# facebookresearch/jepa

Hardware: NVIDIA H100
Metric: clips/sec ViT-L/16 16x224^2 synthetic V-JEPA pre-training step (higher is better)
Workload: dtype bf16

## Files before the change

jepa_b200/csrc/attn_bwd.cu:

```cuda
#include <stdlib.h>

#include "attn_common.cuh"
#include "vjepa_b200.h"

namespace vj {

constexpr int kBwdThreads = 256;
constexpr int kBwdStream = 64;

struct AttnBwdParams {
  const int* cu_seqlens;
  const float* lse2;
  const float* delta;
  __nv_bfloat16* dqkv;
  int H, T;
  float scale, scale_log2;
};

template <int HD>
struct BwdCfg {
  using A = AttnCfg<HD>;
  static constexpr int RES = A::template tile_bytes<128>();
  static constexpr int STR = A::template tile_bytes<kBwdStream>();
  static constexpr int T0 = 0, T1 = RES;
  static constexpr int S_OFF = 2 * RES;
  static constexpr int BAR_OFF = S_OFF + 4 * STR;
  static constexpr int SMEM_BYTES = BAR_OFF + 64 + 1024;
};

__global__ void __launch_bounds__(256) attn_delta_kernel(const __nv_bfloat16* __restrict__ o,
                                                         const __nv_bfloat16* __restrict__ dout,
                                                         float* __restrict__ delta, int T, int H, int HD) {
  const int lane = threadIdx.x & 31;
  const int wpb = blockDim.x >> 5;
  const int D = H * HD;
  const int nvec = D >> 3;
  const int lanes_per_head = HD >> 3;
  for (long long t = (long long)blockIdx.x * wpb + (threadIdx.x >> 5); t < T; t += (long long)gridDim.x * wpb) {
    for (int c = lane; c < ((nvec + 31) / 32) * 32; c += 32) {
      float s = 0.f;
      if (c < nvec) {
        const uint4 a = *reinterpret_cast<const uint4*>(o + t * D + c * 8);
        const uint4 b = *reinterpret_cast<const uint4*>(dout + t * D + c * 8);
        s = bf16_lo(a.x) * bf16_lo(b.x) + bf16_hi(a.x) * bf16_hi(b.x) + bf16_lo(a.y) * bf16_lo(b.y) +
            bf16_hi(a.y) * bf16_hi(b.y) + bf16_lo(a.z) * bf16_lo(b.z) + bf16_hi(a.z) * bf16_hi(b.z) +
            bf16_lo(a.w) * bf16_lo(b.w) + bf16_hi(a.w) * bf16_hi(b.w);
      }
      for (int o2 = lanes_per_head >> 1; o2 > 0; o2 >>= 1) s += __shfl_xor_sync(0xffffffffu, s, o2);
      if (c < nvec && (lane % lanes_per_head) == 0) delta[(long long)((c * 8) / HD) * T + t] = s;
    }
  }
}

template <int HD, bool DKV>
__global__ void __launch_bounds__(kBwdThreads, 1)
attn_bwd_kernel(const __grid_constant__ CUtensorMap tmRes, const __grid_constant__ CUtensorMap tmStr,
                const __grid_constant__ CUtensorMap tmDO, const AttnBwdParams p) {
  using B = BwdCfg<HD>;
  extern __shared__ uint8_t smem_raw[];
  uint8_t* smem = reinterpret_cast<uint8_t*>((reinterpret_cast<uintptr_t>(smem_raw) + 1023) & ~uintptr_t(1023));

  const int seq = blockIdx.y, head = blockIdx.z;
  const int row_begin = p.cu_seqlens[seq];
  const int len = p.cu_seqlens[seq + 1] - row_begin;
  const int t0 = blockIdx.x * 128;
  if (t0 >= len) return;
  const int n_it = (len + kBwdStream - 1) / kBwdStream;
  const int HHD = p.H * HD;

  uint64_t* bars = reinterpret_cast<uint64_t*>(smem + B::BAR_OFF);
  const uint32_t bar_res = smem_u32(bars + 0);
  const uint32_t bar_s0 = smem_u32(bars + 1);
  const uint32_t sT0 = smem_u32(smem + B::T0), sT1 = smem_u32(smem + B::T1), sS = smem_u32(smem + B::S_OFF);

  auto load_stream = [&](int i) {
    const int st = i & 1;
    const uint32_t a = sS + st * 2 * B::STR, b = a + B::STR, bar = bar_s0 + 8 * st;
    const int r0 = row_begin + i * kBwdStream;
    mbar_expect_tx(bar, 2 * B::STR);
    if (DKV) {
      attn_load_tile<HD, kBwdStream>(a, &tmStr, bar, head * HD, r0);
      attn_load_tile<HD, kBwdStream>(b, &tmDO, bar, head * HD, r0);
    } else {
      attn_load_tile<HD, kBwdStream>(a, &tmStr, bar, HHD + head * HD, r0);
      attn_load_tile<HD, kBwdStream>(b, &tmStr, bar, 2 * HHD + head * HD, r0);
    }
  };
  if (threadIdx.x == 0) {
    mbar_init(bar_res, 1);
    mbar_init(bar_s0, 1);
    mbar_init(bar_s0 + 8, 1);
    fence_mbar_init();
    mbar_expect_tx(bar_res, 2 * B::RES);
    if (DKV) {
      attn_load_tile<HD, 128>(sT0, &tmRes, bar_res, HHD + head * HD, row_begin + t0);
      attn_load_tile<HD, 128>(sT1, &tmRes, bar_res, 2 * HHD + head * HD, row_begin + t0);
    } else {
      attn_load_tile<HD, 128>(sT0, &tmRes, bar_res, head * HD, row_begin + t0);
      attn_load_tile<HD, 128>(sT1, &tmDO, bar_res, head * HD, row_begin + t0);
    }
    load_stream(0);
    if (n_it > 1) load_stream(1);
  }
  __syncthreads();

  const int wg = threadIdx.x >> 7;
  const int lane = threadIdx.x & 31;
  const int r = wg * 64 + ((threadIdx.x >> 5) & 3) * 16 + (lane >> 2);
  const float* lse_h = p.lse2 + (long long)head * p.T + row_begin;
  const float* del_h = p.delta + (long long)head * p.T + row_begin;
  float acc0[HD / 2], acc1[HD / 2];
#pragma unroll
  for (int i = 0; i < HD / 2; ++i) { acc0[i] = 0.f; acc1[i] = 0.f; }
  float row_lse[2], row_del[2];
  if (!DKV) {
#pragma unroll
    for (int h = 0; h < 2; ++h) {
      const int q = t0 + r + 8 * h;
      row_lse[h] = q < len ? lse_h[q] : 0.f;
      row_del[h] = q < len ? del_h[q] : 0.f;
    }
  }

  mbar_wait(bar_res, 0);
  for (int i = 0; i < n_it; ++i) {
    const int st = i & 1;
    const uint32_t sa = sS + st * 2 * B::STR, sb = sa + B::STR;
    const int c0 = i * kBwdStream;
    mbar_wait(bar_s0 + 8 * st, (i >> 1) & 1);
    float x[kBwdStream / 2], y[kBwdStream / 2];
    wgmma_fence();
#pragma unroll
    for (int kk = 0; kk < HD / 16; ++kk)
      wgmma_ss<kBwdStream, 0, 0>(x, attn_kmajor_desc<HD, 128>(sT0, wg * 64, kk), attn_kmajor_desc<HD, kBwdStream>(sa, 0, kk),
                                 kk > 0);
#pragma unroll
    for (int kk = 0; kk < HD / 16; ++kk)
      wgmma_ss<kBwdStream, 0, 0>(y, attn_kmajor_desc<HD, 128>(sT1, wg * 64, kk), attn_kmajor_desc<HD, kBwdStream>(sb, 0, kk),
                                 kk > 0);
    wgmma_commit();
    wgmma_wait<0>();
    wgmma_fence_regs(x);
    wgmma_fence_regs(y);

#pragma unroll
    for (int c = 0; c < kBwdStream / 8; ++c)
#pragma unroll
      for (int e = 0; e < 2; ++e) {
        const int col = c0 + 8 * c + 2 * (lane & 3) + e;
        const bool col_ok = col < len;
        float cl = 0.f, cd = 0.f;
        if (DKV && col_ok) { cl = lse_h[col]; cd = del_h[col]; }
#pragma unroll
        for (int h = 0; h < 2; ++h) {
          const float l2 = DKV ? cl : row_lse[h], dl = DKV ? cd : row_del[h];
          float& pv = x[4 * c + 2 * h + e];
          float& dv = y[4 * c + 2 * h + e];
          pv = col_ok ? ex2_approx(fmaf(pv, p.scale_log2, -l2)) : 0.f;
          dv = pv * (dv - dl);
        }
      }

    wgmma_fence_regs(acc0);
    wgmma_fence_regs(acc1);
    wgmma_fence();
#pragma unroll
    for (int kk = 0; kk < kBwdStream / 16; ++kk) {
      uint32_t a[4];
      if (DKV) {
        acc_to_afrag(x, kk, a);
        wgmma_rs<HD, 1>(acc0, a, attn_mnmajor_desc<HD, kBwdStream>(sb, kk), 1);
        acc_to_afrag(y, kk, a);
        wgmma_rs<HD, 1>(acc1, a, attn_mnmajor_desc<HD, kBwdStream>(sa, kk), 1);
      } else {
        acc_to_afrag(y, kk, a);
        wgmma_rs<HD, 1>(acc0, a, attn_mnmajor_desc<HD, kBwdStream>(sa, kk), 1);
      }
    }
    wgmma_commit();
    wgmma_wait<0>();
    wgmma_fence_regs(acc0);
    wgmma_fence_regs(acc1);
    __syncthreads();
    if (threadIdx.x == 0 && i + 2 < n_it) load_stream(i + 2);
  }

  __nv_bfloat16* rows = p.dqkv + (long long)(row_begin + t0) * 3 * HHD + head * HD;
  if (DKV) {
    store_frag_bf16<HD>(acc1, p.scale, rows + HHD, 3LL * HHD, r, len - t0);
    store_frag_bf16<HD>(acc0, 1.0f, rows + 2 * HHD, 3LL * HHD, r, len - t0);
  } else {
    store_frag_bf16<HD>(acc0, p.scale, rows, 3LL * HHD, r, len - t0);
  }
}

template <int HD>
static int launch_attn_bwd(const void* qkv, const void* out, const void* dout, const float* lse2, float* delta,
                           void* dqkv, const int* cu, int nseq, int max_len, int H, int T, float scale, cudaStream_t s) {
  using C = AttnCfg<HD>;
  using B = BwdCfg<HD>;
  CUtensorMap tq128, tq64, tdo128, tdo64;
  const uint64_t W = (uint64_t)3 * H * HD;
  int rc = make_tmap_2d(&tq128, qkv, 0, W, T, W * 2, C::BOX_INNER, 128, C::TMAP_SWIZZLE);
  if (!rc) rc = make_tmap_2d(&tq64, qkv, 0, W, T, W * 2, C::BOX_INNER, kBwdStream, C::TMAP_SWIZZLE);
  if (!rc) rc = make_tmap_2d(&tdo128, dout, 0, (uint64_t)H * HD, T, (uint64_t)H * HD * 2, C::BOX_INNER, 128, C::TMAP_SWIZZLE);
  if (!rc) rc = make_tmap_2d(&tdo64, dout, 0, (uint64_t)H * HD, T, (uint64_t)H * HD * 2, C::BOX_INNER, kBwdStream,
                             C::TMAP_SWIZZLE);
  if (rc) return rc;
  auto kdkv = attn_bwd_kernel<HD, true>;
  auto kdq = attn_bwd_kernel<HD, false>;
  static bool configured = false;
  if (!configured) {
    VJ_CUDA(cudaFuncSetAttribute(kdkv, cudaFuncAttributeMaxDynamicSharedMemorySize, B::SMEM_BYTES));
    VJ_CUDA(cudaFuncSetAttribute(kdq, cudaFuncAttributeMaxDynamicSharedMemorySize, B::SMEM_BYTES));
    configured = true;
  }
  {
    int g = (T + 7) / 8;
    const int cap = num_sms() * 8;
    if (g > cap) g = cap;
    attn_delta_kernel<<<g, 256, 0, s>>>(reinterpret_cast<const __nv_bfloat16*>(out),
                                        reinterpret_cast<const __nv_bfloat16*>(dout), delta, T, H, HD);
    VJ_CUDA(cudaGetLastError());
    vj::count_launch(1);
  }
  AttnBwdParams p;
  p.cu_seqlens = cu; p.lse2 = lse2; p.delta = delta; p.dqkv = reinterpret_cast<__nv_bfloat16*>(dqkv);
  p.H = H; p.T = T; p.scale = scale; p.scale_log2 = scale * 1.4426950408889634f;
  dim3 grid((max_len + 127) / 128, nseq, H);
  kdkv<<<grid, kBwdThreads, B::SMEM_BYTES, s>>>(tq128, tq64, tdo64, p);
  VJ_CUDA(cudaGetLastError());
  kdq<<<grid, kBwdThreads, B::SMEM_BYTES, s>>>(tq128, tq64, tdo128, p);
  VJ_CUDA(cudaGetLastError());
  vj::count_launch(2);
  return 0;
}

// ... 18 lines not shown
```

jepa_b200/csrc/attn_fwd.cu:

```cuda
#include <stdlib.h>

#include "attn_common.cuh"
#include "vjepa_b200.h"

namespace vj {

constexpr int kFwdThreads = 256;
constexpr int kFwdKV = 128;

struct AttnFwdParams {
  const int* cu_seqlens;
  __nv_bfloat16* out;
  float* lse2;
  int H, T;
  long long ld_out;
  float scale_log2;
};

template <int HD>
struct FwdCfg {
  using A = AttnCfg<HD>;
  static constexpr int TILE = A::template tile_bytes<128>();
  static constexpr int Q_OFF = 0;
  static constexpr int K_OFF = TILE;
  static constexpr int V_OFF = 3 * TILE;
  static constexpr int BAR_OFF = 5 * TILE;
  static constexpr int SMEM_BYTES = BAR_OFF + 64 + 1024;
};

template <int HD>
__global__ void __launch_bounds__(kFwdThreads, 1)
attn_fwd_kernel(const __grid_constant__ CUtensorMap tmQKV, const AttnFwdParams p) {
  using F = FwdCfg<HD>;
  extern __shared__ uint8_t smem_raw[];
  uint8_t* smem = reinterpret_cast<uint8_t*>((reinterpret_cast<uintptr_t>(smem_raw) + 1023) & ~uintptr_t(1023));

  const int seq = blockIdx.y, head = blockIdx.z;
  const int row_begin = p.cu_seqlens[seq];
  const int len = p.cu_seqlens[seq + 1] - row_begin;
  const int q0 = blockIdx.x * 128;
  if (q0 >= len) return;
  const int n_kv = (len + kFwdKV - 1) / kFwdKV;

  uint64_t* bars = reinterpret_cast<uint64_t*>(smem + F::BAR_OFF);
  const uint32_t bar_q = smem_u32(bars + 0);
  const uint32_t bar_kv0 = smem_u32(bars + 1);
  const uint32_t sQ = smem_u32(smem + F::Q_OFF), sK = smem_u32(smem + F::K_OFF), sV = smem_u32(smem + F::V_OFF);
  const int HHD = p.H * HD;

  auto load_kv = [&](int j) {
    const int st = j & 1;
    mbar_expect_tx(bar_kv0 + 8 * st, 2 * F::TILE);
    attn_load_tile<HD, 128>(sK + st * F::TILE, &tmQKV, bar_kv0 + 8 * st, HHD + head * HD, row_begin + j * kFwdKV);
    attn_load_tile<HD, 128>(sV + st * F::TILE, &tmQKV, bar_kv0 + 8 * st, 2 * HHD + head * HD, row_begin + j * kFwdKV);
  };
  if (threadIdx.x == 0) {
    mbar_init(bar_q, 1);
    mbar_init(bar_kv0, 1);
    mbar_init(bar_kv0 + 8, 1);
    fence_mbar_init();
    tma_prefetch_desc(&tmQKV);
    mbar_expect_tx(bar_q, F::TILE);
    attn_load_tile<HD, 128>(sQ, &tmQKV, bar_q, head * HD, row_begin + q0);
    load_kv(0);
    if (n_kv > 1) load_kv(1);
  }
  __syncthreads();

  const int wg = threadIdx.x >> 7;
  const int lane = threadIdx.x & 31;
  const int r = wg * 64 + ((threadIdx.x >> 5) & 3) * 16 + (lane >> 2);
  float o[HD / 2];
#pragma unroll
  for (int i = 0; i < HD / 2; ++i) o[i] = 0.f;
  float m_run[2] = {-INFINITY, -INFINITY}, l_run[2] = {0.f, 0.f};

  mbar_wait(bar_q, 0);
  for (int j = 0; j < n_kv; ++j) {
    const int st = j & 1;
    const int valid = min(kFwdKV, len - j * kFwdKV);
    mbar_wait(bar_kv0 + 8 * st, (j >> 1) & 1);
    float s[kFwdKV / 2];
    wgmma_fence();
#pragma unroll
    for (int kk = 0; kk < HD / 16; ++kk)
      wgmma_ss<kFwdKV, 0, 0>(s, attn_kmajor_desc<HD, 128>(sQ, wg * 64, kk),
                             attn_kmajor_desc<HD, 128>(sK + st * F::TILE, 0, kk), kk > 0);
    wgmma_commit();
    wgmma_wait<0>();
    wgmma_fence_regs(s);

    float alpha[2];
#pragma unroll
    for (int h = 0; h < 2; ++h) {
      float mx = -INFINITY;
#pragma unroll
      for (int c = 0; c < kFwdKV / 8; ++c)
#pragma unroll
        for (int e = 0; e < 2; ++e) {
          const int key = 8 * c + 2 * (lane & 3) + e;
          float& v = s[4 * c + 2 * h + e];
          if (key >= valid) v = -INFINITY;
          mx = fmaxf(mx, v);
        }
      mx = quad_max(mx);
      const float m_new = fmaxf(m_run[h], mx);
      alpha[h] = ex2_approx((m_run[h] - m_new) * p.scale_log2);
      m_run[h] = m_new;
      const float moff = m_new * p.scale_log2;
      float sum = 0.f;
#pragma unroll
      for (int c = 0; c < kFwdKV / 8; ++c)
#pragma unroll
        for (int e = 0; e < 2; ++e) {
          float& v = s[4 * c + 2 * h + e];
          v = ex2_approx(fmaf(v, p.scale_log2, -moff));
          sum += v;
        }
      l_run[h] = l_run[h] * alpha[h] + sum;
    }
#pragma unroll
    for (int c = 0; c < HD / 8; ++c) {
      o[4 * c + 0] *= alpha[0]; o[4 * c + 1] *= alpha[0];
      o[4 * c + 2] *= alpha[1]; o[4 * c + 3] *= alpha[1];
    }

    wgmma_fence_regs(o);
    wgmma_fence();
#pragma unroll
    for (int kk = 0; kk < kFwdKV / 16; ++kk) {
      uint32_t a[4];
      acc_to_afrag(s, kk, a);
      wgmma_rs<HD, 1>(o, a, attn_mnmajor_desc<HD, 128>(sV + st * F::TILE, kk), 1);
    }
    wgmma_commit();
    wgmma_wait<0>();
    wgmma_fence_regs(o);
    __syncthreads();
    if (threadIdx.x == 0 && j + 2 < n_kv) load_kv(j + 2);
  }

  float inv[2];
#pragma unroll
  for (int h = 0; h < 2; ++h) {
    const float l = quad_sum(l_run[h]);
    inv[h] = 1.0f / l;
    const int row = q0 + r + 8 * h;
    if ((lane & 3) == 0 && row < len) p.lse2[(long long)head * p.T + row_begin + row] = m_run[h] * p.scale_log2 + log2f(l);
  }
#pragma unroll
  for (int c = 0; c < HD / 8; ++c) {
    o[4 * c + 0] *= inv[0]; o[4 * c + 1] *= inv[0];
    o[4 * c + 2] *= inv[1]; o[4 * c + 3] *= inv[1];
  }
  store_frag_bf16<HD>(o, 1.0f, p.out + (long long)(row_begin + q0) * p.ld_out + head * HD, p.ld_out, r, len - q0);
}

template <int HD>
static int launch_attn_fwd(const void* qkv, void* out, float* lse2, const int* cu, int nseq, int max_len, int H, int T,
                           float scale, cudaStream_t s) {
  using C = AttnCfg<HD>;
  using F = FwdCfg<HD>;
  CUtensorMap tm;
  int rc = make_tmap_2d(&tm, qkv, 0, (uint64_t)3 * H * HD, T, (uint64_t)3 * H * HD * 2, C::BOX_INNER, 128,
                        C::TMAP_SWIZZLE);
  if (rc) return rc;
  auto kern = attn_fwd_kernel<HD>;
  static bool configured = false;
  if (!configured) {
    VJ_CUDA(cudaFuncSetAttribute(kern, cudaFuncAttributeMaxDynamicSharedMemorySize, F::SMEM_BYTES));
    configured = true;
  }
  AttnFwdParams p;
  p.cu_seqlens = cu; p.out = reinterpret_cast<__nv_bfloat16*>(out); p.lse2 = lse2;
  p.H = H; p.T = T; p.ld_out = (long long)H * HD;
  p.scale_log2 = scale * 1.4426950408889634f;
  dim3 grid((max_len + 127) / 128, nseq, H);
  kern<<<grid, kFwdThreads, F::SMEM_BYTES, s>>>(tm, p);
  VJ_CUDA(cudaGetLastError());
  vj::count_launch(1);
  return 0;
}

}

extern "C" int vj_attn_fwd(const void* qkv, void* out, float* lse2, const int* cu_seqlens, int nseq, int max_len,
                           int H, int HD, int T, float scale, void* stream_) {
  using namespace vj;
  cudaStream_t s = reinterpret_cast<cudaStream_t>(stream_);
  VJ_CHECK_ARG(qkv && out && lse2 && cu_seqlens, "vj_attn_fwd: null pointer");
  VJ_CHECK_ARG(nseq > 0 && max_len > 0 && H > 0 && T > 0, "vj_attn_fwd: empty problem");
  VJ_CHECK_ARG((reinterpret_cast<uintptr_t>(qkv) & 15) == 0 && (reinterpret_cast<uintptr_t>(out) & 15) == 0,
               "vj_attn_fwd: pointers must be 16-byte aligned");
// ... 8 lines not shown
```

jepa_b200/csrc/common.cuh:

```cuda
#pragma once

#include <cuda.h>
#include <cuda_bf16.h>
#include <cuda_runtime.h>
#include <stdint.h>

#ifndef VJ_DEVINL
#define VJ_DEVINL __device__ __forceinline__
#endif

namespace vj {

void set_error(const char* fmt, ...);
int cuda_fail(cudaError_t e, const char* what);

#define VJ_CHECK_ARG(cond, ...)                 \
  do {                                          \
    if (!(cond)) {                              \
      vj::set_error(__VA_ARGS__);               \
      return -1;                                \
    }                                           \
  } while (0)

#define VJ_CUDA(expr)                                         \
  do {                                                        \
    cudaError_t _e = (expr);                                  \
    if (_e != cudaSuccess) return vj::cuda_fail(_e, #expr);   \
  } while (0)

int num_sms();
int sm_budget();
void count_launch(int n);

int make_tmap_2d(CUtensorMap* out, const void* ptr, int dtype, uint64_t inner, uint64_t outer,
                 uint64_t ld_bytes, uint32_t box_inner, uint32_t box_outer, int swizzle);

VJ_DEVINL uint32_t smem_u32(const void* p) {
  return static_cast<uint32_t>(__cvta_generic_to_shared(p));
}

VJ_DEVINL void mbar_init(uint32_t bar, uint32_t count) {
  asm volatile("mbarrier.init.shared::cta.b64 [%0], %1;" ::"r"(bar), "r"(count) : "memory");
}
VJ_DEVINL void fence_mbar_init() {
  asm volatile("fence.mbarrier_init.release.cluster;" ::: "memory");
}
VJ_DEVINL void fence_proxy_async_smem() {
  asm volatile("fence.proxy.async.shared::cta;" ::: "memory");
}
VJ_DEVINL void mbar_expect_tx(uint32_t bar, uint32_t bytes) {
  asm volatile("mbarrier.arrive.expect_tx.shared::cta.b64 _, [%0], %1;" ::"r"(bar), "r"(bytes)
               : "memory");
}
VJ_DEVINL void mbar_arrive(uint32_t bar) {
  asm volatile("mbarrier.arrive.shared::cta.b64 _, [%0];" ::"r"(bar) : "memory");
}
VJ_DEVINL bool mbar_try_wait(uint32_t bar, uint32_t parity) {
  uint32_t ok;
  asm volatile(
      "{\n\t.reg .pred p;\n\t"
      "mbarrier.try_wait.parity.shared::cta.b64 p, [%1], %2;\n\t"
      "selp.u32 %0, 1, 0, p;\n\t}"
      : "=r"(ok)
      : "r"(bar), "r"(parity)
      : "memory");
  return ok != 0;
}
VJ_DEVINL void mbar_wait(uint32_t bar, uint32_t parity) {
  while (!mbar_try_wait(bar, parity)) {
  }
}

VJ_DEVINL void tma_prefetch_desc(const CUtensorMap* m) {
  asm volatile("prefetch.tensormap [%0];" ::"l"(reinterpret_cast<uint64_t>(m)) : "memory");
}
VJ_DEVINL void tma_load_2d(uint32_t smem_dst, const CUtensorMap* m, uint32_t bar, int c0, int c1) {
  asm volatile(
      "cp.async.bulk.tensor.2d.shared::cluster.global.mbarrier::complete_tx::bytes [%0], [%1, {%3, %4}], [%2];"
      ::"r"(smem_dst), "l"(reinterpret_cast<uint64_t>(m)), "r"(bar), "r"(c0), "r"(c1)
      : "memory");
}
VJ_DEVINL void tma_store_2d(const CUtensorMap* m, uint32_t smem_src, int c0, int c1) {
  asm volatile("cp.async.bulk.tensor.2d.global.shared::cta.bulk_group [%0, {%2, %3}], [%1];" ::"l"(
                   reinterpret_cast<uint64_t>(m)),
               "r"(smem_src), "r"(c0), "r"(c1)
               : "memory");
}
VJ_DEVINL void tma_reduce_add_2d(const CUtensorMap* m, uint32_t smem_src, int c0, int c1) {
  asm volatile(
      "cp.reduce.async.bulk.tensor.2d.global.shared::cta.add.tile.bulk_group [%0, {%2, %3}], [%1];" ::"l"(
          reinterpret_cast<uint64_t>(m)),
      "r"(smem_src), "r"(c0), "r"(c1)
      : "memory");
}
VJ_DEVINL void tma_commit_group() { asm volatile("cp.async.bulk.commit_group;" ::: "memory"); }
template <int N>
VJ_DEVINL void tma_wait_group_read() {
  asm volatile("cp.async.bulk.wait_group.read %0;" ::"n"(N) : "memory");
}
template <int N>
VJ_DEVINL void tma_wait_group() {
  asm volatile("cp.async.bulk.wait_group %0;" ::"n"(N) : "memory");
}

VJ_DEVINL void sts128(uint32_t addr, const uint4& v) {
  asm volatile("st.shared.v4.b32 [%0], {%1, %2, %3, %4};" ::"r"(addr), "r"(v.x), "r"(v.y), "r"(v.z), "r"(v.w) : "memory");
}
VJ_DEVINL void sts128f(uint32_t addr, const float4& v) {
  asm volatile("st.shared.v4.f32 [%0], {%1, %2, %3, %4};" ::"r"(addr), "f"(v.x), "f"(v.y), "f"(v.z), "f"(v.w) : "memory");
}
VJ_DEVINL uint4 lds128(uint32_t addr) {
  uint4 v;
  asm volatile("ld.shared.v4.b32 {%0, %1, %2, %3}, [%4];" : "=r"(v.x), "=r"(v.y), "=r"(v.z), "=r"(v.w) : "r"(addr) : "memory");
  return v;
}
VJ_DEVINL float4 lds128f(uint32_t addr) {
  float4 v;
  asm volatile("ld.shared.v4.f32 {%0, %1, %2, %3}, [%4];" : "=f"(v.x), "=f"(v.y), "=f"(v.z), "=f"(v.w) : "r"(addr) : "memory");
  return v;
}
VJ_DEVINL void sts32f(uint32_t addr, float v) { asm volatile("st.shared.f32 [%0], %1;" ::"r"(addr), "f"(v) : "memory"); }
VJ_DEVINL float lds32f(uint32_t addr) {
  float v;
  asm volatile("ld.shared.f32 %0, [%1];" : "=f"(v) : "r"(addr) : "memory");
// ... 51 lines not shown
```

jepa_b200/csrc/gemm.cu:

```cuda

#include <stdlib.h>

#include "common.cuh"
#include "vjepa_b200.h"
#include "wgmma.cuh"

namespace vj {

constexpr int BM = 128;
constexpr int BK = 64;
constexpr int kGemmThreads = 384;
constexpr int kPromoteKB = 4;

struct GemmParams {
  int M, N, K;
  int tiles_m, tiles_n, split_k, kb_total, kb_per_split;
  int stream_k;
  long long sk_chunk;
  const float* bias;
  int epi;
  const void* aux;
  long long ldaux;
  const int* aux_rowmap;
  int aux_period;
// ... 23 lines not shown
  WorkCursor c;
  if (p.stream_k) {
    const long long total_kb = (long long)p.tiles_m * p.tiles_n * p.kb_total;
    c.cur = (long long)blockIdx.x * p.sk_chunk;
    c.end = min(total_kb, c.cur + p.sk_chunk);
  } else {
    c.cur = blockIdx.x;
    c.end = (long long)p.tiles_m * p.tiles_n * p.split_k;
  }
  return c;
}
VJ_DEVINL bool work_next(const GemmParams& p, WorkCursor& c, int& t, int& kb0, int& kb1) {
  if (c.cur >= c.end) return false;
  if (p.stream_k) {
    t = int(c.cur / p.kb_total);
    kb0 = int(c.cur - (long long)t * p.kb_total);
    const long long take = min((long long)(p.kb_total - kb0), c.end - c.cur);
    kb1 = kb0 + int(take);
    c.cur += take;
  } else {
    const int tiles = p.tiles_m * p.tiles_n;
    const int split = int(c.cur / tiles);
    t = int(c.cur - (long long)split * tiles);
    kb0 = split * p.kb_per_split;
    kb1 = min(p.kb_total, kb0 + p.kb_per_split);
    c.cur += gridDim.x;
  }
  return true;
}

VJ_DEVINL float erf_as(float x) {
  const float ax = fabsf(x);
  const float t = __fdividef(1.0f, fmaf(0.3275911f, ax, 1.0f));
  float poly = fmaf(1.061405429f, t, -1.453152027f);
  poly = fmaf(poly, t, 1.421413741f);
  poly = fmaf(poly, t, -0.284496736f);
  poly = fmaf(poly, t, 0.254829592f);
  poly *= t;
  const float r = 1.0f - poly * __expf(-ax * ax);
  return copysignf(r, x);
}
VJ_DEVINL float gelu_and_grad(float x, float& d) {
  const float cdf = 0.5f * (1.0f + erf_as(x * 0.70710678118654752f));
  const float pdf = 0.39894228040143268f * __expf(-0.5f * x * x);
  d = fmaf(x, pdf, cdf);
  return x * cdf;
}
VJ_DEVINL float gelu_grad_fast(float x) {
  float d;
  gelu_and_grad(x, d);
  return d;
}

VJ_DEVINL void setmaxnreg_dec40() { asm volatile("setmaxnreg.dec.sync.aligned.u32 40;"); }
VJ_DEVINL void setmaxnreg_inc232() { asm volatile("setmaxnreg.inc.sync.aligned.u32 232;"); }

template <int BN, bool A_MN, bool B_MN, bool OUT_F32, int EPI, bool AUX32>
__global__ void __launch_bounds__(kGemmThreads, 1)
gemm_kernel(const __grid_constant__ CUtensorMap tmA, const __grid_constant__ CUtensorMap tmB, const GemmParams p) {
  constexpr bool kUsesAux = (EPI == VJ_EPI_ADD || EPI == VJ_EPI_DGELU || EPI == VJ_EPI_MUL);
  using Cfg = GemmCfg<BN>;
  constexpr int STAGES = Cfg::STAGES;
  extern __shared__ uint8_t smem_raw[];
  uint8_t* smem = reinterpret_cast<uint8_t*>((reinterpret_cast<uintptr_t>(smem_raw) + 1023) & ~uintptr_t(1023));
  uint64_t* bars = reinterpret_cast<uint64_t*>(smem + Cfg::BAR_OFF);
  const uint32_t full0 = smem_u32(bars);
  const uint32_t empty0 = smem_u32(bars + STAGES);
  const int wg = threadIdx.x >> 7;

  if (threadIdx.x == 0) {
    for (int s = 0; s < STAGES; ++s) {
      mbar_init(full0 + 8 * s, 1);
      mbar_init(empty0 + 8 * s, 8);
    }
    fence_mbar_init();
    tma_prefetch_desc(&tmA);
    tma_prefetch_desc(&tmB);
  }
  __syncthreads();

  if (wg == 0) {
    setmaxnreg_dec40();
    if (threadIdx.x == 0) {
      int stage = 0;
      uint32_t phase = 0;
      WorkCursor wc = work_begin(p);
      int t, kb0, kb1;
      while (work_next(p, wc, t, kb0, kb1)) {
        const int m0 = (t / p.tiles_n) * BM;
        const int n0 = (t % p.tiles_n) * BN;
        for (int kb = kb0; kb < kb1; ++kb) {
          mbar_wait(empty0 + 8 * stage, phase ^ 1);
          const uint32_t sa = smem_u32(smem + stage * Cfg::STAGE_BYTES);
          const uint32_t sb = sa + Cfg::A_BYTES;
          const uint32_t fb = full0 + 8 * stage;
          mbar_expect_tx(fb, Cfg::STAGE_BYTES);
          const int k0 = kb * BK;
          if (!A_MN) {
            tma_load_2d(sa, &tmA, fb, k0, m0);
          } else {
#pragma unroll
            for (int j = 0; j < BM / 64; ++j) tma_load_2d(sa + j * 8192, &tmA, fb, m0 + 64 * j, k0);
          }
          if (!B_MN) {
            tma_load_2d(sb, &tmB, fb, k0, n0);
          } else {
#pragma unroll
            for (int j = 0; j < BN / 64; ++j) tma_load_2d(sb + j * 8192, &tmB, fb, n0 + 64 * j, k0);
          }
          if (++stage == STAGES) {
            stage = 0;
            phase ^= 1;
          }
        }
      }
    }
    return;
  }

  setmaxnreg_inc232();
  const int cw = wg - 1;
  const int warp_in_wg = (threadIdx.x >> 5) & 3;
  const int lane = threadIdx.x & 31;
  constexpr bool kPromote = A_MN && B_MN;
  static_assert(!kPromote || BN <= 128, "promoted accumulation needs two accumulator sets in registers");
  int stage = 0;
  uint32_t phase = 0;
  float acc[BN / 2];
  float part[kPromote ? BN / 2 : 1];
  WorkCursor wc = work_begin(p);
  int t, kb0, kb1;
  while (work_next(p, wc, t, kb0, kb1)) {
    const int m0 = (t / p.tiles_n) * BM;
    const int n0 = (t % p.tiles_n) * BN;
    if constexpr (kPromote) {
#pragma unroll
      for (int i = 0; i < BN / 2; ++i) acc[i] = 0.f;
    }
    int prev = -1;
    for (int kb = kb0; kb < kb1; ++kb) {
      mbar_wait(full0 + 8 * stage, phase);
      const uint32_t sa = smem_u32(smem + stage * Cfg::STAGE_BYTES) + cw * 8192;
      const uint32_t sb = smem_u32(smem + stage * Cfg::STAGE_BYTES) + Cfg::A_BYTES;
      const uint64_t da0 = A_MN ? make_smem_desc(sa, 8192, 1024, 1) : make_smem_desc(sa, 16, 1024, 1);
      const uint64_t db0 = B_MN ? make_smem_desc(sb, 8192, 1024, 1) : make_smem_desc(sb, 16, 1024, 1);
      if constexpr (kPromote) {
        const bool group_first = (kb - kb0) % kPromoteKB == 0;
        const bool group_last = (kb - kb0) % kPromoteKB == kPromoteKB - 1 || kb + 1 == kb1;
        wgmma_fence_regs(part);
        wgmma_fence();
#pragma unroll
        for (int kk = 0; kk < BK / 16; ++kk)
          wgmma_ss<BN, 1, 1>(part, da0 + ((kk * 2048) >> 4), db0 + ((kk * 2048) >> 4), (!group_first || kk > 0) ? 1 : 0);
        wgmma_commit();
        if (group_last) {
          wgmma_wait<0>();
          wgmma_fence_regs(part);
#pragma unroll
          for (int i = 0; i < BN / 2; ++i) acc[i] += part[i];
        } else {
          wgmma_wait<1>();
        }
      } else {
        wgmma_fence_regs(acc);
        wgmma_fence();
#pragma unroll
        for (int kk = 0; kk < BK / 16; ++kk) {
          const uint32_t koa = A_MN ? kk * 2048 : kk * 32, kob = B_MN ? kk * 2048 : kk * 32;
          wgmma_ss<BN, A_MN ? 1 : 0, B_MN ? 1 : 0>(acc, da0 + (koa >> 4), db0 + (kob >> 4), (kb > kb0 || kk > 0) ? 1 : 0);
        }
        wgmma_commit();
        wgmma_wait<1>();
        wgmma_fence_regs(acc);
// ... 200 lines not shown
```

jepa_b200/csrc/wgmma.cuh:

```cuda
#pragma once
#include <stdint.h>

namespace vj {

__device__ __forceinline__ void wgmma_fence() { asm volatile("wgmma.fence.sync.aligned;" ::: "memory"); }
__device__ __forceinline__ void wgmma_commit() { asm volatile("wgmma.commit_group.sync.aligned;" ::: "memory"); }
template <int N>
__device__ __forceinline__ void wgmma_wait() { asm volatile("wgmma.wait_group.sync.aligned %0;" ::"n"(N) : "memory"); }
template <int R>
__device__ __forceinline__ void wgmma_fence_regs(float (&d)[R]) {
#pragma unroll
  for (int i = 0; i < R; ++i) asm volatile("" : "+f"(d[i])::"memory");
}

template <int N, int TA, int TB>
__device__ __forceinline__ void wgmma_ss(float (&d)[N / 2], uint64_t da, uint64_t db, int scale_d);
template <int N, int TB>
__device__ __forceinline__ void wgmma_rs(float (&d)[N / 2], const uint32_t (&a)[4], uint64_t db, int scale_d);

#define VJ_WGMMA_SS_64(TA, TB)                                                                                   \
  template <>                                                                                                    \
  __device__ __forceinline__ void wgmma_ss<64, TA, TB>(float (&d)[32], uint64_t da, uint64_t db, int scale_d) {   \
    asm volatile("{\n.reg .pred p;\nsetp.ne.b32 p, %34, 0;\n"                                                   \
                 "wgmma.mma_async.sync.aligned.m64n64k16.f32.bf16.bf16 {%0, %1, %2, %3, %4, %5, %6, %7, %8, %9, %10, %11, %12, %13, %14, %15, %16, %17, %18, %19, %20, %21, %22, %23, %24, %25, %26, %27, %28, %29, %30, %31}, %32, %33, p, 1, 1, " #TA ", " #TB ";\n}" \
                 : "+f"(d[0]), "+f"(d[1]), "+f"(d[2]), "+f"(d[3]), "+f"(d[4]), "+f"(d[5]), "+f"(d[6]), "+f"(d[7]), "+f"(d[8]), "+f"(d[9]), "+f"(d[10]), "+f"(d[11]), "+f"(d[12]), "+f"(d[13]), "+f"(d[14]), "+f"(d[15]), "+f"(d[16]), "+f"(d[17]), "+f"(d[18]), "+f"(d[19]), "+f"(d[20]), "+f"(d[21]), "+f"(d[22]), "+f"(d[23]), "+f"(d[24]), "+f"(d[25]), "+f"(d[26]), "+f"(d[27]), "+f"(d[28]), "+f"(d[29]), "+f"(d[30]), "+f"(d[31])                                                                                        \
                 : "l"(da), "l"(db), "r"(scale_d));                                                              \
  }
VJ_WGMMA_SS_64(0, 0)
VJ_WGMMA_SS_64(0, 1)
VJ_WGMMA_SS_64(1, 1)
#undef VJ_WGMMA_SS_64

#define VJ_WGMMA_SS_128(TA, TB)                                                                                   \
  template <>                                                                                                    \
  __device__ __forceinline__ void wgmma_ss<128, TA, TB>(float (&d)[64], uint64_t da, uint64_t db, int scale_d) {   \
    asm volatile("{\n.reg .pred p;\nsetp.ne.b32 p, %66, 0;\n"                                                   \
                 "wgmma.mma_async.sync.aligned.m64n128k16.f32.bf16.bf16 {%0, %1, %2, %3, %4, %5, %6, %7, %8, %9, %10, %11, %12, %13, %14, %15, %16, %17, %18, %19, %20, %21, %22, %23, %24, %25, %26, %27, %28, %29, %30, %31, %32, %33, %34, %35, %36, %37, %38, %39, %40, %41, %42, %43, %44, %45, %46, %47, %48, %49, %50, %51, %52, %53, %54, %55, %56, %57, %58, %59, %60, %61, %62, %63}, %64, %65, p, 1, 1, " #TA ", " #TB ";\n}" \
                 : "+f"(d[0]), "+f"(d[1]), "+f"(d[2]), "+f"(d[3]), "+f"(d[4]), "+f"(d[5]), "+f"(d[6]), "+f"(d[7]), "+f"(d[8]), "+f"(d[9]), "+f"(d[10]), "+f"(d[11]), "+f"(d[12]), "+f"(d[13]), "+f"(d[14]), "+f"(d[15]), "+f"(d[16]), "+f"(d[17]), "+f"(d[18]), "+f"(d[19]), "+f"(d[20]), "+f"(d[21]), "+f"(d[22]), "+f"(d[23]), "+f"(d[24]), "+f"(d[25]), "+f"(d[26]), "+f"(d[27]), "+f"(d[28]), "+f"(d[29]), "+f"(d[30]), "+f"(d[31]), "+f"(d[32]), "+f"(d[33]), "+f"(d[34]), "+f"(d[35]), "+f"(d[36]), "+f"(d[37]), "+f"(d[38]), "+f"(d[39]), "+f"(d[40]), "+f"(d[41]), "+f"(d[42]), "+f"(d[43]), "+f"(d[44]), "+f"(d[45]), "+f"(d[46]), "+f"(d[47]), "+f"(d[48]), "+f"(d[49]), "+f"(d[50]), "+f"(d[51]), "+f"(d[52]), "+f"(d[53]), "+f"(d[54]), "+f"(d[55]), "+f"(d[56]), "+f"(d[57]), "+f"(d[58]), "+f"(d[59]), "+f"(d[60]), "+f"(d[61]), "+f"(d[62]), "+f"(d[63])                                                                                        \
                 : "l"(da), "l"(db), "r"(scale_d));                                                              \
  }
VJ_WGMMA_SS_128(0, 0)
VJ_WGMMA_SS_128(0, 1)
VJ_WGMMA_SS_128(1, 1)
#undef VJ_WGMMA_SS_128

#define VJ_WGMMA_SS_256(TA, TB)                                                                                   \
  template <>                                                                                                    \
  __device__ __forceinline__ void wgmma_ss<256, TA, TB>(float (&d)[128], uint64_t da, uint64_t db, int scale_d) {   \
    asm volatile("{\n.reg .pred p;\nsetp.ne.b32 p, %130, 0;\n"                                                   \
                 "wgmma.mma_async.sync.aligned.m64n256k16.f32.bf16.bf16 {%0, %1, %2, %3, %4, %5, %6, %7, %8, %9, %10, %11, %12, %13, %14, %15, %16, %17, %18, %19, %20, %21, %22, %23, %24, %25, %26, %27, %28, %29, %30, %31, %32, %33, %34, %35, %36, %37, %38, %39, %40, %41, %42, %43, %44, %45, %46, %47, %48, %49, %50, %51, %52, %53, %54, %55, %56, %57, %58, %59, %60, %61, %62, %63, %64, %65, %66, %67, %68, %69, %70, %71, %72, %73, %74, %75, %76, %77, %78, %79, %80, %81, %82, %83, %84, %85, %86, %87, %88, %89, %90, %91, %92, %93, %94, %95, %96, %97, %98, %99, %100, %101, %102, %103, %104, %105, %106, %107, %108, %109, %110, %111, %112, %113, %114, %115, %116, %117, %118, %119, %120, %121, %122, %123, %124, %125, %126, %127}, %128, %129, p, 1, 1, " #TA ", " #TB ";\n}" \
                 : "+f"(d[0]), "+f"(d[1]), "+f"(d[2]), "+f"(d[3]), "+f"(d[4]), "+f"(d[5]), "+f"(d[6]), "+f"(d[7]), "+f"(d[8]), "+f"(d[9]), "+f"(d[10]), "+f"(d[11]), "+f"(d[12]), "+f"(d[13]), "+f"(d[14]), "+f"(d[15]), "+f"(d[16]), "+f"(d[17]), "+f"(d[18]), "+f"(d[19]), "+f"(d[20]), "+f"(d[21]), "+f"(d[22]), "+f"(d[23]), "+f"(d[24]), "+f"(d[25]), "+f"(d[26]), "+f"(d[27]), "+f"(d[28]), "+f"(d[29]), "+f"(d[30]), "+f"(d[31]), "+f"(d[32]), "+f"(d[33]), "+f"(d[34]), "+f"(d[35]), "+f"(d[36]), "+f"(d[37]), "+f"(d[38]), "+f"(d[39]), "+f"(d[40]), "+f"(d[41]), "+f"(d[42]), "+f"(d[43]), "+f"(d[44]), "+f"(d[45]), "+f"(d[46]), "+f"(d[47]), "+f"(d[48]), "+f"(d[49]), "+f"(d[50]), "+f"(d[51]), "+f"(d[52]), "+f"(d[53]), "+f"(d[54]), "+f"(d[55]), "+f"(d[56]), "+f"(d[57]), "+f"(d[58]), "+f"(d[59]), "+f"(d[60]), "+f"(d[61]), "+f"(d[62]), "+f"(d[63]), "+f"(d[64]), "+f"(d[65]), "+f"(d[66]), "+f"(d[67]), "+f"(d[68]), "+f"(d[69]), "+f"(d[70]), "+f"(d[71]), "+f"(d[72]), "+f"(d[73]), "+f"(d[74]), "+f"(d[75]), "+f"(d[76]), "+f"(d[77]), "+f"(d[78]), "+f"(d[79]), "+f"(d[80]), "+f"(d[81]), "+f"(d[82]), "+f"(d[83]), "+f"(d[84]), "+f"(d[85]), "+f"(d[86]), "+f"(d[87]), "+f"(d[88]), "+f"(d[89]), "+f"(d[90]), "+f"(d[91]), "+f"(d[92]), "+f"(d[93]), "+f"(d[94]), "+f"(d[95]), "+f"(d[96]), "+f"(d[97]), "+f"(d[98]), "+f"(d[99]), "+f"(d[100]), "+f"(d[101]), "+f"(d[102]), "+f"(d[103]), "+f"(d[104]), "+f"(d[105]), "+f"(d[106]), "+f"(d[107]), "+f"(d[108]), "+f"(d[109]), "+f"(d[110]), "+f"(d[111]), "+f"(d[112]), "+f"(d[113]), "+f"(d[114]), "+f"(d[115]), "+f"(d[116]), "+f"(d[117]), "+f"(d[118]), "+f"(d[119]), "+f"(d[120]), "+f"(d[121]), "+f"(d[122]), "+f"(d[123]), "+f"(d[124]), "+f"(d[125]), "+f"(d[126]), "+f"(d[127])                                                                                        \
                 : "l"(da), "l"(db), "r"(scale_d));                                                              \
  }
VJ_WGMMA_SS_256(0, 0)
VJ_WGMMA_SS_256(0, 1)
VJ_WGMMA_SS_256(1, 1)
#undef VJ_WGMMA_SS_256

template <>
__device__ __forceinline__ void wgmma_rs<32, 1>(float (&d)[16], const uint32_t (&a)[4], uint64_t db, int scale_d) {
  asm volatile("{\n.reg .pred p;\nsetp.ne.b32 p, %21, 0;\n"
               "wgmma.mma_async.sync.aligned.m64n32k16.f32.bf16.bf16 {%0, %1, %2, %3, %4, %5, %6, %7, %8, %9, %10, %11, %12, %13, %14, %15}, {%16, %17, %18, %19}, %20, p, 1, 1, 1;\n}"
               : "+f"(d[0]), "+f"(d[1]), "+f"(d[2]), "+f"(d[3]), "+f"(d[4]), "+f"(d[5]), "+f"(d[6]), "+f"(d[7]), "+f"(d[8]), "+f"(d[9]), "+f"(d[10]), "+f"(d[11]), "+f"(d[12]), "+f"(d[13]), "+f"(d[14]), "+f"(d[15])
               : "r"(a[0]), "r"(a[1]), "r"(a[2]), "r"(a[3]), "l"(db), "r"(scale_d));
}
// ... 19 lines not shown
```

Measured before the change: 98.39.

## Warp-specialize attention kernels with producer warpgroup, 3-stage mbarrier ring, and ping-pong

Both attention forward and backward kernels now use a dedicated producer warpgroup that issues TMA loads into a 3-stage ring with full/empty mbarriers, replacing the block-wide __syncthreads refill. Register budgets are rebalanced with setmaxnreg. The forward kernel overlaps the next QK^T wgmma with the current PV wgmma and alternates the two consumer warpgroups on tensor cores via named barriers. The backward dK/dV path stages per-column lse/delta into shared memory from the producer warp instead of reading them from global memory in the inner loop. This adds complexity, uses more shared memory, and carries a risk of barrier or phase bugs.

```diff
diff --git a/jepa_b200/csrc/attn_bwd.cu b/jepa_b200/csrc/attn_bwd.cu
--- a/jepa_b200/csrc/attn_bwd.cu
+++ b/jepa_b200/csrc/attn_bwd.cu
@@ -5,8 +5,9 @@
 
 namespace vj {
 
-constexpr int kBwdThreads = 256;
+constexpr int kBwdThreads = 384;
 constexpr int kBwdStream = 64;
+constexpr int kBwdStages = 3;
 
 struct AttnBwdParams {
   const int* cu_seqlens;
@@ -24,8 +25,11 @@
   static constexpr int STR = A::template tile_bytes<kBwdStream>();
   static constexpr int T0 = 0, T1 = RES;
   static constexpr int S_OFF = 2 * RES;
-  static constexpr int BAR_OFF = S_OFF + 4 * STR;
-  static constexpr int SMEM_BYTES = BAR_OFF + 64 + 1024;
+  static constexpr int STAT_OFF = S_OFF + kBwdStages * 2 * STR;
+  static constexpr int STAT = 2 * kBwdStream * 4;
+  static constexpr int BAR_OFF = STAT_OFF + kBwdStages * STAT;
+  static constexpr int SMEM_BYTES = BAR_OFF + 8 * (1 + 2 * kBwdStages) + 1024;
+  static_assert(SMEM_BYTES <= 232448, "attention backward shared memory budget exceeded");
 };
 
 __global__ void __launch_bounds__(256) attn_delta_kernel(const __nv_bfloat16* __restrict__ o,
@@ -70,45 +74,72 @@
 
   uint64_t* bars = reinterpret_cast<uint64_t*>(smem + B::BAR_OFF);
   const uint32_t bar_res = smem_u32(bars + 0);
-  const uint32_t bar_s0 = smem_u32(bars + 1);
+  const uint32_t full0 = smem_u32(bars + 1);
+  const uint32_t empty0 = smem_u32(bars + 1 + kBwdStages);
   const uint32_t sT0 = smem_u32(smem + B::T0), sT1 = smem_u32(smem + B::T1), sS = smem_u32(smem + B::S_OFF);
-
-  auto load_stream = [&](int i) {
-    const int st = i & 1;
-    const uint32_t a = sS + st * 2 * B::STR, b = a + B::STR, bar = bar_s0 + 8 * st;
-    const int r0 = row_begin + i * kBwdStream;
-    mbar_expect_tx(bar, 2 * B::STR);
-    if (DKV) {
-      attn_load_tile<HD, kBwdStream>(a, &tmStr, bar, head * HD, r0);
-      attn_load_tile<HD, kBwdStream>(b, &tmDO, bar, head * HD, r0);
-    } else {
-      attn_load_tile<HD, kBwdStream>(a, &tmStr, bar, HHD + head * HD, r0);
-      attn_load_tile<HD, kBwdStream>(b, &tmStr, bar, 2 * HHD + head * HD, r0);
-    }
-  };
+  const uint32_t sStat = smem_u32(smem + B::STAT_OFF);
+  const float* lse_h = p.lse2 + (long long)head * p.T + row_begin;
+  const float* del_h = p.delta + (long long)head * p.T + row_begin;
+  const int wg = threadIdx.x >> 7;
+  const int lane = threadIdx.x & 31;
+
   if (threadIdx.x == 0) {
     mbar_init(bar_res, 1);
-    mbar_init(bar_s0, 1);
-    mbar_init(bar_s0 + 8, 1);
+    for (int st = 0; st < kBwdStages; ++st) {
+      mbar_init(full0 + 8 * st, DKV ? 32 : 1);
+      mbar_init(empty0 + 8 * st, 8);
+    }
     fence_mbar_init();
-    mbar_expect_tx(bar_res, 2 * B::RES);
-    if (DKV) {
-      attn_load_tile<HD, 128>(sT0, &tmRes, bar_res, HHD + head * HD, row_begin + t0);
-      attn_load_tile<HD, 128>(sT1, &tmRes, bar_res, 2 * HHD + head * HD, row_begin + t0);
-    } else {
-      attn_load_tile<HD, 128>(sT0, &tmRes, bar_res, head * HD, row_begin + t0);
-      attn_load_tile<HD, 128>(sT1, &tmDO, bar_res, head * HD, row_begin + t0);
-    }
-    load_stream(0);
-    if (n_it > 1) load_stream(1);
   }
   __syncthreads();
 
-  const int wg = threadIdx.x >> 7;
-  const int lane = threadIdx.x & 31;
-  const int r = wg * 64 + ((threadIdx.x >> 5) & 3) * 16 + (lane >> 2);
-  const float* lse_h = p.lse2 + (long long)head * p.T + row_begin;
-  const float* del_h = p.delta + (long long)head * p.T + row_begin;
+  if (wg == 0) {
+    setmaxnreg_dec<40>();
+    if (threadIdx.x < 32) {
+      if (lane == 0) {
+        mbar_expect_tx(bar_res, 2 * B::RES);
+        if (DKV) {
+          attn_load_tile<HD, 128>(sT0, &tmRes, bar_res, HHD + head * HD, row_begin + t0);
+          attn_load_tile<HD, 128>(sT1, &tmRes, bar_res, 2 * HHD + head * HD, row_begin + t0);
+        } else {
+          attn_load_tile<HD, 128>(sT0, &tmRes, bar_res, head * HD, row_begin + t0);
+          attn_load_tile<HD, 128>(sT1, &tmDO, bar_res, head * HD, row_begin + t0);
+        }
+      }
+      for (int i = 0; i < n_it; ++i) {
+        const int st = i % kBwdStages;
+        const uint32_t a = sS + st * 2 * B::STR, b = a + B::STR, bar = full0 + 8 * st;
+        const int c0 = i * kBwdStream;
+        mbar_wait(empty0 + 8 * st, ((i / kBwdStages) & 1) ^ 1);
+        if (DKV) {
+#pragma unroll
+          for (int k = 0; k < kBwdStream / 32; ++k) {
+            const int col = c0 + 32 * k + lane;
+            const uint32_t dst = sStat + st * B::STAT + (32 * k + lane) * 4;
+            sts32f(dst, col < len ? lse_h[col] : 0.f);
+            sts32f(dst + B::STAT / 2, col < len ? del_h[col] : 0.f);
+          }
+        }
+        if (lane == 0) {
+          mbar_expect_tx(bar, 2 * B::STR);
+          if (DKV) {
+            attn_load_tile<HD, kBwdStream>(a, &tmStr, bar, head * HD, row_begin + c0);
+            attn_load_tile<HD, kBwdStream>(b, &tmDO, bar, head * HD, row_begin + c0);
+          } else {
+            attn_load_tile<HD, kBwdStream>(a, &tmStr, bar, HHD + head * HD, row_begin + c0);
+            attn_load_tile<HD, kBwdStream>(b, &tmStr, bar, 2 * HHD + head * HD, row_begin + c0);
+          }
+        } else if (DKV) {
+          mbar_arrive(bar);
+        }
+      }
+    }
+    return;
+  }
+
+  setmaxnreg_inc<232>();
+  const int cw = wg - 1;
+  const int r = cw * 64 + ((threadIdx.x >> 5) & 3) * 16 + (lane >> 2);
   float acc0[HD / 2], acc1[HD / 2];
 #pragma unroll
   for (int i = 0; i < HD / 2; ++i) { acc0[i] = 0.f; acc1[i] = 0.f; }
@@ -121,22 +152,21 @@
       row_del[h] = q < len ? del_h[q] : 0.f;
     }
   }
-
   mbar_wait(bar_res, 0);
   for (int i = 0; i < n_it; ++i) {
-    const int st = i & 1;
+    const int st = i % kBwdStages;
     const uint32_t sa = sS + st * 2 * B::STR, sb = sa + B::STR;
     const int c0 = i * kBwdStream;
-    mbar_wait(bar_s0 + 8 * st, (i >> 1) & 1);
+    mbar_wait(full0 + 8 * st, (i / kBwdStages) & 1);
     float x[kBwdStream / 2], y[kBwdStream / 2];
     wgmma_fence();
 #pragma unroll
     for (int kk = 0; kk < HD / 16; ++kk)
-      wgmma_ss<kBwdStream, 0, 0>(x, attn_kmajor_desc<HD, 128>(sT0, wg * 64, kk), attn_kmajor_desc<HD, kBwdStream>(sa, 0, kk),
+      wgmma_ss<kBwdStream, 0, 0>(x, attn_kmajor_desc<HD, 128>(sT0, cw * 64, kk), attn_kmajor_desc<HD, kBwdStream>(sa, 0, kk),
                                  kk > 0);
 #pragma unroll
     for (int kk = 0; kk < HD / 16; ++kk)
-      wgmma_ss<kBwdStream, 0, 0>(y, attn_kmajor_desc<HD, 128>(sT1, wg * 64, kk), attn_kmajor_desc<HD, kBwdStream>(sb, 0, kk),
+      wgmma_ss<kBwdStream, 0, 0>(y, attn_kmajor_desc<HD, 128>(sT1, cw * 64, kk), attn_kmajor_desc<HD, kBwdStream>(sb, 0, kk),
                                  kk > 0);
     wgmma_commit();
     wgmma_wait<0>();
@@ -147,10 +177,13 @@
     for (int c = 0; c < kBwdStream / 8; ++c)
 #pragma unroll
       for (int e = 0; e < 2; ++e) {
-        const int col = c0 + 8 * c + 2 * (lane & 3) + e;
-        const bool col_ok = col < len;
+        const int col = 8 * c + 2 * (lane & 3) + e;
+        const bool col_ok = c0 + col < len;
         float cl = 0.f, cd = 0.f;
-        if (DKV && col_ok) { cl = lse_h[col]; cd = del_h[col]; }
+        if (DKV) {
+          cl = lds32f(sStat + st * B::STAT + col * 4);
+          cd = lds32f(sStat + st * B::STAT + B::STAT / 2 + col * 4);
+        }
 #pragma unroll
         for (int h = 0; h < 2; ++h) {
           const float l2 = DKV ? cl : row_lse[h], dl = DKV ? cd : row_del[h];
@@ -181,8 +214,8 @@
     wgmma_wait<0>();
     wgmma_fence_regs(acc0);
     wgmma_fence_regs(acc1);
-    __syncthreads();
-    if (threadIdx.x == 0 && i + 2 < n_it) load_stream(i + 2);
+    __syncwarp();
+    if (lane == 0) mbar_arrive(empty0 + 8 * st);
   }
 
   __nv_bfloat16* rows = p.dqkv + (long long)(row_begin + t0) * 3 * HHD + head * HD;
diff --git a/jepa_b200/csrc/attn_fwd.cu b/jepa_b200/csrc/attn_fwd.cu
--- a/jepa_b200/csrc/attn_fwd.cu
+++ b/jepa_b200/csrc/attn_fwd.cu
@@ -5,8 +5,9 @@
 
 namespace vj {
 
-constexpr int kFwdThreads = 256;
+constexpr int kFwdThreads = 384;
 constexpr int kFwdKV = 128;
+constexpr int kFwdStages = 3;
 
 struct AttnFwdParams {
   const int* cu_seqlens;
@@ -23,10 +24,14 @@
   static constexpr int TILE = A::template tile_bytes<128>();
   static constexpr int Q_OFF = 0;
   static constexpr int K_OFF = TILE;
-  static constexpr int V_OFF = 3 * TILE;
-  static constexpr int BAR_OFF = 5 * TILE;
-  static constexpr int SMEM_BYTES = BAR_OFF + 64 + 1024;
+  static constexpr int V_OFF = K_OFF + kFwdStages * TILE;
+  static constexpr int BAR_OFF = V_OFF + kFwdStages * TILE;
+  static constexpr int SMEM_BYTES = BAR_OFF + 8 * (1 + 2 * kFwdStages) + 1024;
+  static_assert(SMEM_BYTES <= 232448, "attention forward shared memory budget exceeded");
 };
+
+VJ_DEVINL void pingpong_wait_turn(int cw) { named_bar_sync(1 + cw, 256); }
+VJ_DEVINL void pingpong_pass_turn(int cw) { named_bar_arrive(2 - cw, 256); }
 
 template <int HD>
 __global__ void __launch_bounds__(kFwdThreads, 1)
@@ -44,65 +49,84 @@
 
   uint64_t* bars = reinterpret_cast<uint64_t*>(smem + F::BAR_OFF);
   const uint32_t bar_q = smem_u32(bars + 0);
-  const uint32_t bar_kv0 = smem_u32(bars + 1);
+  const uint32_t full0 = smem_u32(bars + 1);
+  const uint32_t empty0 = smem_u32(bars + 1 + kFwdStages);
   const uint32_t sQ = smem_u32(smem + F::Q_OFF), sK = smem_u32(smem + F::K_OFF), sV = smem_u32(smem + F::V_OFF);
   const int HHD = p.H * HD;
-
-  auto load_kv = [&](int j) {
-    const int st = j & 1;
-    mbar_expect_tx(bar_kv0 + 8 * st, 2 * F::TILE);
-    attn_load_tile<HD, 128>(sK + st * F::TILE, &tmQKV, bar_kv0 + 8 * st, HHD + head * HD, row_begin + j * kFwdKV);
-    attn_load_tile<HD, 128>(sV + st * F::TILE, &tmQKV, bar_kv0 + 8 * st, 2 * HHD + head * HD, row_begin + j * kFwdKV);
-  };
+  const int wg = threadIdx.x >> 7;
+
   if (threadIdx.x == 0) {
     mbar_init(bar_q, 1);
-    mbar_init(bar_kv0, 1);
-    mbar_init(bar_kv0 + 8, 1);
+    for (int st = 0; st < kFwdStages; ++st) {
+      mbar_init(full0 + 8 * st, 1);
+      mbar_init(empty0 + 8 * st, 8);
+    }
     fence_mbar_init();
     tma_prefetch_desc(&tmQKV);
-    mbar_expect_tx(bar_q, F::TILE);
-    attn_load_tile<HD, 128>(sQ, &tmQKV, bar_q, head * HD, row_begin + q0);
-    load_kv(0);
-    if (n_kv > 1) load_kv(1);
   }
   __syncthreads();
 
-  const int wg = threadIdx.x >> 7;
+  if (wg == 0) {
+    setmaxnreg_dec<40>();
+    if (threadIdx.x == 0) {
+      mbar_expect_tx(bar_q, F::TILE);
+      attn_load_tile<HD, 128>(sQ, &tmQKV, bar_q, head * HD, row_begin + q0);
+      for (int j = 0; j < n_kv; ++j) {
+        const int st = j % kFwdStages;
+        mbar_wait(empty0 + 8 * st, ((j / kFwdStages) & 1) ^ 1);
+        const uint32_t fb = full0 + 8 * st;
+        mbar_expect_tx(fb, 2 * F::TILE);
+        attn_load_tile<HD, 128>(sK + st * F::TILE, &tmQKV, fb, HHD + head * HD, row_begin + j * kFwdKV);
+        attn_load_tile<HD, 128>(sV + st * F::TILE, &tmQKV, fb, 2 * HHD + head * HD, row_begin + j * kFwdKV);
+      }
+    }
+    return;
+  }
+
+  setmaxnreg_inc<232>();
+  const int cw = wg - 1;
   const int lane = threadIdx.x & 31;
-  const int r = wg * 64 + ((threadIdx.x >> 5) & 3) * 16 + (lane >> 2);
+  const int r = cw * 64 + ((threadIdx.x >> 5) & 3) * 16 + (lane >> 2);
   float o[HD / 2];
 #pragma unroll
   for (int i = 0; i < HD / 2; ++i) o[i] = 0.f;
   float m_run[2] = {-INFINITY, -INFINITY}, l_run[2] = {0.f, 0.f};
-
-  mbar_wait(bar_q, 0);
-  for (int j = 0; j < n_kv; ++j) {
-    const int st = j & 1;
-    const int valid = min(kFwdKV, len - j * kFwdKV);
-    mbar_wait(bar_kv0 + 8 * st, (j >> 1) & 1);
-    float s[kFwdKV / 2];
-    wgmma_fence();
+  float s[kFwdKV / 2];
+  uint32_t pf[kFwdKV / 16][4];
+  if (cw == 1) pingpong_pass_turn(cw);
+
+  auto issue_s = [&](int st) {
 #pragma unroll
     for (int kk = 0; kk < HD / 16; ++kk)
-      wgmma_ss<kFwdKV, 0, 0>(s, attn_kmajor_desc<HD, 128>(sQ, wg * 64, kk),
+      wgmma_ss<kFwdKV, 0, 0>(s, attn_kmajor_desc<HD, 128>(sQ, cw * 64, kk),
                              attn_kmajor_desc<HD, 128>(sK + st * F::TILE, 0, kk), kk > 0);
     wgmma_commit();
-    wgmma_wait<0>();
-    wgmma_fence_regs(s);
-
-    float alpha[2];
+  };
+  auto issue_pv = [&](int st) {
+#pragma unroll
+    for (int kk = 0; kk < kFwdKV / 16; ++kk) wgmma_rs<HD, 1>(o, pf[kk], attn_mnmajor_desc<HD, 128>(sV + st * F::TILE, kk), 1);
+    wgmma_commit();
+  };
+  auto release = [&](int st) {
+    __syncwarp();
+    if (lane == 0) mbar_arrive(empty0 + 8 * st);
+  };
+  auto softmax = [&](int j, float (&alpha)[2]) {
+    const int valid = len - j * kFwdKV;
+    if (valid < kFwdKV) {
+#pragma unroll
+      for (int c = 0; c < kFwdKV / 8; ++c)
+#pragma unroll
+        for (int e = 0; e < 4; ++e)
+          if (8 * c + 2 * (lane & 3) + (e & 1) >= valid) s[4 * c + e] = -INFINITY;
+    }
 #pragma unroll
     for (int h = 0; h < 2; ++h) {
       float mx = -INFINITY;
 #pragma unroll
       for (int c = 0; c < kFwdKV / 8; ++c)
 #pragma unroll
-        for (int e = 0; e < 2; ++e) {
-          const int key = 8 * c + 2 * (lane & 3) + e;
-          float& v = s[4 * c + 2 * h + e];
-          if (key >= valid) v = -INFINITY;
-          mx = fmaxf(mx, v);
-        }
+        for (int e = 0; e < 2; ++e) mx = fmaxf(mx, s[4 * c + 2 * h + e]);
       mx = quad_max(mx);
       const float m_new = fmaxf(m_run[h], mx);
       alpha[h] = ex2_approx((m_run[h] - m_new) * p.scale_log2);
@@ -119,26 +143,59 @@
         }
       l_run[h] = l_run[h] * alpha[h] + sum;
     }
+  };
+  auto rescale_o = [&](const float (&alpha)[2]) {
 #pragma unroll
     for (int c = 0; c < HD / 8; ++c) {
       o[4 * c + 0] *= alpha[0]; o[4 * c + 1] *= alpha[0];
       o[4 * c + 2] *= alpha[1]; o[4 * c + 3] *= alpha[1];
     }
-
+  };
+  auto pack_p = [&]() {
+#pragma unroll
+    for (int kk = 0; kk < kFwdKV / 16; ++kk) acc_to_afrag(s, kk, pf[kk]);
+  };
+
+  mbar_wait(bar_q, 0);
+  float alpha[2];
+  pingpong_wait_turn(cw);
+  mbar_wait(full0, 0);
+  wgmma_fence();
+  issue_s(0);
+  pingpong_pass_turn(cw);
+  wgmma_wait<0>();
+  wgmma_fence_regs(s);
+  softmax(0, alpha);
+  rescale_o(alpha);
+  pack_p();
+  for (int j = 1; j < n_kv; ++j) {
+    const int st = j % kFwdStages, st_prev = (j - 1) % kFwdStages;
+    pingpong_wait_turn(cw);
+    mbar_wait(full0 + 8 * st, (j / kFwdStages) & 1);
     wgmma_fence_regs(o);
     wgmma_fence();
-#pragma unroll
-    for (int kk = 0; kk < kFwdKV / 16; ++kk) {
-      uint32_t a[4];
-      acc_to_afrag(s, kk, a);
-      wgmma_rs<HD, 1>(o, a, attn_mnmajor_desc<HD, 128>(sV + st * F::TILE, kk), 1);
-    }
-    wgmma_commit();
+    issue_s(st);
+    issue_pv(st_prev);
+    pingpong_pass_turn(cw);
+    wgmma_wait<1>();
+    wgmma_fence_regs(s);
+    softmax(j, alpha);
     wgmma_wait<0>();
     wgmma_fence_regs(o);
-    __syncthreads();
-    if (threadIdx.x == 0 && j + 2 < n_kv) load_kv(j + 2);
-  }
+    wgmma_fence_regs(pf);
+    release(st_prev);
+    rescale_o(alpha);
+    pack_p();
+  }
+  pingpong_wait_turn(cw);
+  wgmma_fence_regs(o);
+  wgmma_fence();
+  issue_pv((n_kv - 1) % kFwdStages);
+  pingpong_pass_turn(cw);
+  wgmma_wait<0>();
+  wgmma_fence_regs(o);
+  wgmma_fence_regs(pf);
+  if (cw == 0) pingpong_wait_turn(cw);
 
   float inv[2];
 #pragma unroll
diff --git a/jepa_b200/csrc/common.cuh b/jepa_b200/csrc/common.cuh
--- a/jepa_b200/csrc/common.cuh
+++ b/jepa_b200/csrc/common.cuh
@@ -70,6 +70,18 @@
   while (!mbar_try_wait(bar, parity)) {
   }
 }
+
+VJ_DEVINL void named_bar_sync(int id, int threads) {
+  asm volatile("bar.sync %0, %1;" ::"r"(id), "r"(threads) : "memory");
+}
+VJ_DEVINL void named_bar_arrive(int id, int threads) {
+  asm volatile("bar.arrive %0, %1;" ::"r"(id), "r"(threads) : "memory");
+}
+
+template <int N>
+VJ_DEVINL void setmaxnreg_dec() { asm volatile("setmaxnreg.dec.sync.aligned.u32 %0;" ::"n"(N)); }
+template <int N>
+VJ_DEVINL void setmaxnreg_inc() { asm volatile("setmaxnreg.inc.sync.aligned.u32 %0;" ::"n"(N)); }
 
 VJ_DEVINL void tma_prefetch_desc(const CUtensorMap* m) {
   asm volatile("prefetch.tensormap [%0];" ::"l"(reinterpret_cast<uint64_t>(m)) : "memory");
diff --git a/jepa_b200/csrc/gemm.cu b/jepa_b200/csrc/gemm.cu
--- a/jepa_b200/csrc/gemm.cu
+++ b/jepa_b200/csrc/gemm.cu
@@ -99,9 +99,6 @@
   return d;
 }
 
-VJ_DEVINL void setmaxnreg_dec40() { asm volatile("setmaxnreg.dec.sync.aligned.u32 40;"); }
-VJ_DEVINL void setmaxnreg_inc232() { asm volatile("setmaxnreg.inc.sync.aligned.u32 232;"); }
-
 template <int BN, bool A_MN, bool B_MN, bool OUT_F32, int EPI, bool AUX32>
 __global__ void __launch_bounds__(kGemmThreads, 1)
 gemm_kernel(const __grid_constant__ CUtensorMap tmA, const __grid_constant__ CUtensorMap tmB, const GemmParams p) {
@@ -127,7 +124,7 @@
   __syncthreads();
 
   if (wg == 0) {
-    setmaxnreg_dec40();
+    setmaxnreg_dec<40>();
     if (threadIdx.x == 0) {
       int stage = 0;
       uint32_t phase = 0;
@@ -165,7 +162,7 @@
     return;
   }
 
-  setmaxnreg_inc232();
+  setmaxnreg_inc<232>();
   const int cw = wg - 1;
   const int warp_in_wg = (threadIdx.x >> 5) & 3;
   const int lane = threadIdx.x & 31;
diff --git a/jepa_b200/csrc/wgmma.cuh b/jepa_b200/csrc/wgmma.cuh
--- a/jepa_b200/csrc/wgmma.cuh
+++ b/jepa_b200/csrc/wgmma.cuh
@@ -11,6 +11,13 @@
 __device__ __forceinline__ void wgmma_fence_regs(float (&d)[R]) {
 #pragma unroll
   for (int i = 0; i < R; ++i) asm volatile("" : "+f"(d[i])::"memory");
+}
+template <int K>
+__device__ __forceinline__ void wgmma_fence_regs(uint32_t (&a)[K][4]) {
+#pragma unroll
+  for (int k = 0; k < K; ++k)
+#pragma unroll
+    for (int i = 0; i < 4; ++i) asm volatile("" : "+r"(a[k][i])::"memory");
 }
 
 template <int N, int TA, int TB>
```

Result: faster. 102.3, median of 6 (+4.0%).
